# helenypzhang/Subspace-Multimodal-Learning

Hardware: AMD Instinct MI355X
Metric: bags/sec fwd+bwd, DeformCrossTransMIL N=10k x 512 (higher is better)
Workload: dtype f32

## Files before the change

subspace-multimodal-learning_amd/csrc/cpb_regions.h:

```cpp
#pragma once
#include <type_traits>
#include "deform_common.h"
#include "deform16_types.h"

namespace {

constexpr int RG_MAX_KEYS = 16384;
constexpr int RG_G = 1024;
constexpr int RG_SUB = 8;
constexpr int RG_SUBC = (RG_SUB + 1) * (RG_SUB + 1);
constexpr int RG_SUBCAP = 16384;
constexpr int RG_EDGES = 1 << 15;
constexpr unsigned RG_E_SUB0 = 4096u, RG_E_EDGE0 = RG_E_SUB0 + 16384u;
constexpr int RG_CANDCAP = 1 << 18;
constexpr int RG_HASH = 16384;
constexpr int RG_RCAP = 4096;
constexpr int RG_LCAP = 2048;
constexpr unsigned RG_NONE = 0xFFFFu;
constexpr unsigned long long RG_EMPTY = ~0ull;
constexpr unsigned RG_K_REGION = 0u << 30, RG_K_EDGE = 1u << 30, RG_K_SUB = 2u << 30, RG_K_MLP = 3u << 30, RG_PAYLOAD = 0x3FFFFFFFu;

struct RegionHeader {
  unsigned n_sub, n_edge, n_cand, n_regions, n_keys, overflow;
  unsigned n_cand1, pad0;
// ... 714 lines not shown
        for (int r = 0; r < 16; ++r) LTb[(size_t)(j0 + acc_row(r, hf)) * 32 + c] = s[r];
      } else {
#pragma unroll
        for (int r = 0; r < 16; ++r) {
          const int key = acc_row(r, hf);
          if (key < nk) LTb[(size_t)(j0 + key) * 32 + c] = s[r];
        }
      }
    }
    if constexpr (SAVE && !F32) {
      if (nk == KT) {
#pragma unroll
        for (int r = 0; r < 16; r += 2) {
          unsigned w = pack_score(s[r], s[r + 1]);
          if (dc.thresh) w = stash_keep16x2(w, keepbits >> r);
          const unsigned lo = w & 0xFFFFu, hi = w >> 16;
          LTb[(size_t)(j0 + acc_row(r, hf)) * 32 + c] = (u16)lo;
          LTb[(size_t)(j0 + acc_row(r + 1, hf)) * 32 + c] = (u16)hi;
          s[r] = score_of(lo); s[r + 1] = score_of(hi);
        }
      } else {
#pragma unroll
        for (int r = 0; r < 16; r += 2) {
          const unsigned w = pack_score(s[r], s[r + 1]);
          unsigned lo = w & 0xFFFFu, hi = w >> 16;
          const int k0 = acc_row(r, hf), k1 = acc_row(r + 1, hf);
          if (dc.thresh) {
            if (k0 < nk) lo = stash_keep16(lo, (keepbits >> r) & 1u);
            if (k1 < nk) hi = stash_keep16(hi, (keepbits >> (r + 1)) & 1u);
          }
          if (k0 < nk) { LTb[(size_t)(j0 + k0) * 32 + c] = (u16)lo; s[r] = score_of(lo); }
          if (k1 < nk) { LTb[(size_t)(j0 + k1) * 32 + c] = (u16)hi; s[r + 1] = score_of(hi); }
        }
      }
      tmax = -INFINITY;
#pragma unroll
      for (int r = 0; r < 16; ++r) tmax = fmaxf(tmax, s[r]);
    }
    fetch_kv(j0 + KT);
    if (kt + 1 < ntiles) step1((kt + 1) & 1);
    tmax = xhalf_max(tmax);
    const float m_new = fmaxf(m_run, tmax);
    const float alpha = sexp(m_run - m_new);
    float psum = 0.f;
#pragma unroll
    for (int r = 0; r < 16; ++r) {
      const float p = sexp(s[r] - m_new);
      psum += p;
      s[r] = p;
    }
    if (dc.thresh) {
#pragma unroll
      for (int r = 0; r < 16; ++r) s[r] *= ((keepbits >> r) & 1u) ? dc.keep_scale : 0.f;
    }
    l_run = l_run * alpha + psum;
    m_run = m_new;
#pragma unroll
    for (int r = 0; r < 16; ++r) { oacc0[r] *= alpha; oacc1[r] *= alpha; }
    if (kt + 1 < ntiles) step2a();
    __builtin_amdgcn_sched_barrier(0);

#pragma unroll
    for (int kb = 0; kb < 2; ++kb) {
      float p8[8];
#pragma unroll
      for (int j = 0; j < 8; ++j) p8[j] = s[8 * kb + j];
      const int ro = (16 * kb + 4 * hf + trq) * FTLD + trc;
      if constexpr (F32) {
        half8 ph, pl;
        split8(p8, ph, pl);
        const half8 vh0 = lds_frag_tr_h(&Vp[0][ro], &Vp[0][ro + 8 * FTLD]), vl0 = lds_frag_tr_h(&Vp[1][ro], &Vp[1][ro + 8 * FTLD]);
        const half8 vh1 = lds_frag_tr_h(&Vp[0][ro + 32], &Vp[0][ro + 32 + 8 * FTLD]), vl1 = lds_frag_tr_h(&Vp[1][ro + 32], &Vp[1][ro + 32 + 8 * FTLD]);
        oacc0 = mfma16(vl0, ph, oacc0); oacc0 = mfma16(vh0, pl, oacc0); oacc0 = mfma16(vh0, ph, oacc0);
        oacc1 = mfma16(vl1, ph, oacc1); oacc1 = mfma16(vh1, pl, oacc1); oacc1 = mfma16(vh1, ph, oacc1);
      } else {
        const vec8 pt = cvt8<T16>(p8);
        oacc0 = mma(frag_tr<T16>(&V16[ro], &V16[ro + 8 * FTLD]), pt, oacc0);
        oacc1 = mma(frag_tr<T16>(&V16[ro + 32], &V16[ro + 32 + 8 * FTLD]), pt, oacc1);
      }
    }
  }

  l_run = xhalf_sum(l_run);
  const float inv = 1.f / l_run;
  if (qvalid) {
    float* op = O + ((size_t)b * N + qi) * HD + h * DH;
#pragma unroll
    for (int rg = 0; rg < 4; ++rg) {
      const int d = 8 * rg + 4 * hf;
      *reinterpret_cast<float4*>(op + d) = make_float4(oacc0[4 * rg] * inv, oacc0[4 * rg + 1] * inv, oacc0[4 * rg + 2] * inv, oacc0[4 * rg + 3] * inv);
      *reinterpret_cast<float4*>(op + 32 + d) = make_float4(oacc1[4 * rg] * inv, oacc1[4 * rg + 1] * inv, oacc1[4 * rg + 2] * inv, oacc1[4 * rg + 3] * inv);
    }
    if (hf == 0) LSE[(size_t)(b * H + h) * N + qi] = m_run + logf(l_run);
  }
}

__device__ __forceinline__ long long region_fix(float v, double S) {
  return __double_as_longlong(fma((double)v, S, 6755399441055744.0)) - 0x4338000000000000ll;
}
struct RegionScale { double S; int e; };
__device__ __forceinline__ RegionScale region_scale(unsigned amax_bits, int kbits) {
  RegionScale r;
  r.e = amax_bits ? (int)((amax_bits >> 23) & 0xFFu) - 126 : 0;
  r.S = __longlong_as_double((long long)(1023 + kbits - r.e) << 52);
  return r;
}
constexpr int RG_GRAD = CPB_SLAB;

struct RegionBwdLds {
  unsigned long long hist[RG_LCAP * 3];
  unsigned long long grad[RG_GRAD];
  float2 reg2[RG_LCAP];
  float w2t[CH * CH], w2r[CH * CH];
  float2 dvs[16][64];
};

template <typename DS, bool MH = false>
__global__ __launch_bounds__(768) void cpb_region_bwd_kernel(
    const DS* __restrict__ dLT, const unsigned short* __restrict__ RID, const float* __restrict__ VS, const float* __restrict__ GQ,
    CpbParams cp, RegionView rv, const unsigned* __restrict__ AMAX, unsigned long long* __restrict__ HIST, unsigned long long* __restrict__ GRAD,
    float* __restrict__ dvs_slab, int N, int J, int H, int NST, int nkb, int nkbg, int chunks, int wpk, int tiles_per_chunk, int kbits, int shift,
    int lcap, int G) {
  extern __shared__ __attribute__((aligned(16))) unsigned char smem_raw[];
  RegionBwdLds& L = *reinterpret_cast<RegionBwdLds*>(smem_raw);
  const int tid = threadIdx.x, lane = tid & 63, c = lane & 31, hf = lane >> 5;
  const int wave = __builtin_amdgcn_readfirstlane(tid >> 6);
  const int b = blockIdx.z, h = blockIdx.y, chunk = blockIdx.x % chunks, grp = blockIdx.x / chunks;
  const int nthreads = blockDim.x;
  const int hpg = MH ? H / G : 1, g = MH ? h / hpg : h, oi = MH ? h - g * hpg : 0;
  const float4* __restrict__ regs = (MH && oi) ? region_reg1(rv.hdr) : rv.reg;
  HIST += MH ? (size_t)oi * RG_RCAP * 3 : 0;
  GRAD += MH ? (size_t)oi * RG_GRAD : 0;
  {
    const int nreg = min((int)rv.hdr->n_regions, lcap);
    for (int i = tid; i < RG_LCAP * 3; i += nthreads) L.hist[i] = 0ull;
    for (int i = tid; i < RG_GRAD; i += nthreads) L.grad[i] = 0ull;
    for (int i = tid; i < nreg; i += nthreads) { const float4 r = regs[i]; L.reg2[i] = make_float2(r.x, r.y); }
    for (int i = tid; i < CH * CH; i += nthreads) { const float w = cp.w2[i]; L.w2r[i] = w; L.w2t[(i & 31) * CH + (i >> 5)] = w; }
  }
  __syncthreads();
  const RegionScale sc = region_scale(*AMAX, kbits);
  const double Sg = __longlong_as_double(__double_as_longlong(sc.S) - ((long long)shift << 52));
  const CoopMlp mlp{cp.w1[c * 2], cp.w1[c * 2 + 1], cp.b1[c], cp.b2[c], cp.w3[oi * CH + c], cp.b3[oi], L.w2t, L.w2r};
  float big;
  asm("s_mov_b32 %0, 0x71800000" : "=s"(big));

  const int kb = grp * nkbg + __builtin_amdgcn_readfirstlane(wave % nkbg), tslot = __builtin_amdgcn_readfirstlane(wave / nkbg);
  const int key = lane * nkb + kb;
  const bool kvalid = key < J && kb < nkb;
  const int keyc = min(key, J - 1);
  const size_t vrow = (size_t)(b * (MH ? G : H) + g) * J;
  const float vs0 = VS[(vrow + keyc) * 2], vs1 = VS[(vrow + keyc) * 2 + 1];
  const int ntq = (N + QT - 1) / QT;
  const int t_begin = chunk * tiles_per_chunk, t_end = min(t_begin + tiles_per_chunk, ntq);
  float dv0 = 0.f, dv1 = 0.f;
  unsigned bad = 0u;
  unsigned cur = ~0u;
  float r0 = 0.f, r1 = 0.f, r2 = 0.f, u0 = 0.f, u1 = 0.f;
  typedef __attribute__((address_space(3))) unsigned long long lds_u64;
  typedef __attribute__((address_space(1))) unsigned long long glb_u64;
  lds_u64* const hist_l = (lds_u64*)L.hist;
  glb_u64* const hist_g = (glb_u64*)HIST;
  auto flush = [&]() {
    if (cur < (unsigned)lcap) {
      const float2 a = L.reg2[cur];
      dv0 = fmaf(-a.x, u0, dv0); dv1 = fmaf(-a.y, u1, dv1);
      lds_u64* hp = hist_l + cur * 3;
      __hip_atomic_fetch_add(hp, (unsigned long long)region_fix(r0, sc.S), __ATOMIC_RELAXED, __HIP_MEMORY_SCOPE_WORKGROUP);
      __hip_atomic_fetch_add(hp + 1, (unsigned long long)region_fix(r1, sc.S), __ATOMIC_RELAXED, __HIP_MEMORY_SCOPE_WORKGROUP);
      __hip_atomic_fetch_add(hp + 2, (unsigned long long)region_fix(r2, sc.S), __ATOMIC_RELAXED, __HIP_MEMORY_SCOPE_WORKGROUP);
    } else if (cur < (unsigned)RG_NONE) {
      const float4 a = regs[cur];
      dv0 = fmaf(-a.x, u0, dv0); dv1 = fmaf(-a.y, u1, dv1);
      glb_u64* hp = hist_g + cur * 3;
      __hip_atomic_fetch_add(hp, (unsigned long long)region_fix(r0, Sg), __ATOMIC_RELAXED, __HIP_MEMORY_SCOPE_AGENT);
      __hip_atomic_fetch_add(hp + 1, (unsigned long long)region_fix(r1, Sg), __ATOMIC_RELAXED, __HIP_MEMORY_SCOPE_AGENT);
      __hip_atomic_fetch_add(hp + 2, (unsigned long long)region_fix(r2, Sg), __ATOMIC_RELAXED, __HIP_MEMORY_SCOPE_AGENT);
    }
  };

  constexpr bool DS32 = std::is_same<DS, float>::value;
  float4 dbn[DS32 ? 8 : 4];
  uint4 ridn[4];
  float2 gqn;
  auto fetch = [&](int tile) {
    const size_t row = ((size_t)(b * H + h) * NST + (size_t)tile * QT) * J + (size_t)keyc * 32;
    const float4* dp = reinterpret_cast<const float4*>(dLT + row);
    const uint4* rp = reinterpret_cast<const uint4*>(RID + row);
#pragma unroll
    for (int i = 0; i < (DS32 ? 8 : 4); ++i) dbn[i] = dp[i];
#pragma unroll
    for (int i = 0; i < 4; ++i) ridn[i] = rp[i];
    gqn = reinterpret_cast<const float2*>(GQ)[min(tile * QT + c, N - 1)];
  };
  if (t_begin + tslot < t_end) fetch(t_begin + tslot);
  for (int tile = t_begin + tslot; tile < t_end; tile += wpk) {
    const int q0 = __builtin_amdgcn_readfirstlane(tile) * QT;
    const int nq = min(QT, N - q0);
    float dbr[32];
    unsigned ridw[16];
    if constexpr (DS32) {
#pragma unroll
      for (int i = 0; i < 8; ++i) { dbr[4 * i] = dbn[i].x; dbr[4 * i + 1] = dbn[i].y; dbr[4 * i + 2] = dbn[i].z; dbr[4 * i + 3] = dbn[i].w; }
    } else {
#pragma unroll
      for (int i = 0; i < 4; ++i) {
        const unsigned w4[4] = {__float_as_uint(dbn[i].x), __float_as_uint(dbn[i].y), __float_as_uint(dbn[i].z), __float_as_uint(dbn[i].w)};
#pragma unroll
        for (int j = 0; j < 4; ++j) { dbr[8 * i + 2 * j] = bf_lo(w4[j]); dbr[8 * i + 2 * j + 1] = bf_hi(w4[j]); }
      }
    }
#pragma unroll
    for (int i = 0; i < 4; ++i) { ridw[4 * i] = ridn[i].x; ridw[4 * i + 1] = ridn[i].y; ridw[4 * i + 2] = ridn[i].z; ridw[4 * i + 3] = ridn[i].w; }
    if (!kvalid) {
#pragma unroll
      for (int i = 0; i < 16; ++i) ridw[i] = 0xFFFFFFFFu;
    }
    const int gqx = __float_as_int(gqn.x), gqy = __float_as_int(gqn.y);
    if (tile + wpk < t_end) fetch(tile + wpk);
    unsigned nonemask = 0u;
    int gy_prev = 0;
    float p1 = 0.f, s1 = 0.f;
#pragma unroll
    for (int q = 0; q < 32; ++q) {
      if (q < nq) {
        const int gxb = __builtin_amdgcn_readlane(gqx, q), gyb = __builtin_amdgcn_readlane(gqy, q);
        const float d0 = __int_as_float(gxb) - vs0;
        const float p0 = slog1p(d0), s0 = dpos_of<false>(d0, big);
        if (q == 0 || gyb != gy_prev) {
          const float d1 = __int_as_float(gyb) - vs1;
          p1 = slog1p(d1); s1 = dpos_of<false>(d1, big);
          gy_prev = gyb;
        }
        const unsigned id = (ridw[q >> 1] >> (16 * (q & 1))) & 0xFFFFu;
        const float dbv = dbr[q];
        if constexpr (MH) {
          unsigned ub = __float_as_uint(dbv);
          asm("" : "+v"(ub));
          bad |= ((ub & 0x7F800000u) == 0x7F800000u) ? 1u : 0u;
        }
        if (id != cur) {
          flush();
          if (id == RG_NONE) { nonemask |= 1u << q; cur = ~0u; }
          else cur = id;
          r0 = 0.f; r1 = 0.f; r2 = 0.f; u0 = 0.f; u1 = 0.f;
        }
        r0 += dbv; r1 = fmaf(dbv, p0, r1); r2 = fmaf(dbv, p1, r2);
        u0 = fmaf(dbv, s0, u0); u1 = fmaf(dbv, s1, u1);
      }
    }
    if (!kvalid) nonemask = 0u;
    for (unsigned long long todo = __ballot(nonemask != 0u); todo; todo &= todo - 1) {
      const int l = __ffsll((long long)todo) - 1;
      const float v0 = __shfl(vs0, l), v1 = __shfl(vs1, l);
      const int kl = __shfl(keyc, l);
      const DS* drow = dLT + ((size_t)(b * H + h) * NST + (size_t)q0) * J + (size_t)kl * 32;
      for (unsigned m = (unsigned)__shfl((int)nonemask, l); m; m &= m - 1) {
        const int q = __ffs((int)m) - 1;
        const float d0 = GQ[(size_t)(q0 + q) * 2] - v0, d1 = GQ[(size_t)(q0 + q) * 2 + 1] - v1;
        const float pp0 = slog1p(d0), pp1 = slog1p(d1);
        float dbl;
        if constexpr (DS32) dbl = drow[q];
        else dbl = tof<__bf16>((unsigned)drow[q]);
        float h1; bool on2;
        (void)coop_mlp_fwd(mlp, pp0, pp1, c, h1, on2);
        float x2 = mlp.b2;
#pragma unroll 8
        for (int i = 0; i < CH; ++i) x2 = fmaf(mlp.w2t[i * CH + c], __shfl(h1, i), x2);
        const float g2 = on2 ? mlp.w3 : 0.f;
        float c1 = 0.f;
#pragma unroll 8
        for (int o = 0; o < CH; ++o) c1 = fmaf(mlp.w2r[o * CH + c], __shfl(g2, o), c1);
        c1 = h1 > 0.f ? c1 : 0.f;
        const float dp0 = coop_sum32(c1 * mlp.w1x), dp1 = coop_sum32(c1 * mlp.w1y);
        if (lane == l) {
          dv0 = fmaf(-dbl * dp0, dpos_of<false>(d0, big), dv0);
          dv1 = fmaf(-dbl * dp1, dpos_of<false>(d1, big), dv1);
        }
        for (int ii = 0; ii < 16; ++ii) {
          const int i = 16 * hf + ii;
          const float hi = __shfl(h1, i);
          atomicAdd(&L.grad[c * CH + i], (unsigned long long)region_fix(dbl * g2 * hi, sc.S));
        }
        if (hf == 0) {
          atomicAdd(&L.grad[1024 + 2 * c], (unsigned long long)region_fix(dbl * c1 * pp0, sc.S));
          atomicAdd(&L.grad[1024 + 2 * c + 1], (unsigned long long)region_fix(dbl * c1 * pp1, sc.S));
          atomicAdd(&L.grad[1024 + 64 + c], (unsigned long long)region_fix(dbl * c1, sc.S));
          atomicAdd(&L.grad[1024 + 96 + c], (unsigned long long)region_fix(dbl * g2, sc.S));
          atomicAdd(&L.grad[1024 + 128 + c], (unsigned long long)region_fix(on2 ? dbl * x2 : 0.f, sc.S));
          if (c == 0) atomicAdd(&L.grad[1024 + 160], (unsigned long long)region_fix(dbl, sc.S));
        }
      }
    }
  }
  flush();
  if constexpr (MH) {
    if (__ballot(kvalid && bad != 0u) && lane == 0) atomicOr(const_cast<unsigned*>(AMAX) + 1, 1u);
  }
  L.dvs[wave][lane] = make_float2(dv0, dv1);
  __syncthreads();
  if (wave < nkbg && kvalid) {
    float2 sum = L.dvs[wave][lane];
    for (int s2 = 1; s2 < wpk; ++s2) { const float2 t = L.dvs[wave + s2 * nkbg][lane]; sum.x += t.x; sum.y += t.y; }
    reinterpret_cast<float2*>(dvs_slab)[((size_t)chunk * gridDim.z * gridDim.y + (size_t)(b * H + h)) * J + key] = sum;
  }
  const long long half = shift > 0 ? (1ll << (shift - 1)) : 0ll;
  for (int i = tid; i < RG_LCAP * 3; i += nthreads) {
    const long long v = (long long)L.hist[i];
    if (v != 0ll) atomicAdd(&HIST[i], (unsigned long long)((v + half) >> shift));
  }
  for (int i = tid; i < RG_GRAD; i += nthreads) {
    const long long v = (long long)L.grad[i];
    if (v != 0ll) atomicAdd(&GRAD[i], (unsigned long long)((v + half) >> shift));
  }
}
template <typename T>
__global__ __launch_bounds__(256) void region_dvs_reduce_kernel(const T* __restrict__ slab, T* __restrict__ dVS, int H, int J, int chunks) {
  const int j = blockIdx.x * blockDim.x + threadIdx.x;
  if (j >= J) return;
  const int G = gridDim.y, hpg = H / G;
  const size_t per = (size_t)gridDim.z * H * J, first = ((size_t)blockIdx.z * H + blockIdx.y * hpg) * J + j;
  T s = slab[first];
  for (int k = 0; k < chunks; ++k)
    for (int o = k ? 0 : 1; o < hpg; ++o) s += slab[(size_t)k * per + first + (size_t)o * J];
  dVS[((size_t)blockIdx.z * G + blockIdx.y) * J + j] = s;
}

constexpr int RG_FIN = 32, RG_HPG = 2;
template <typename Geo, int HPG>
struct RegionSlab {
  static constexpr int W2 = 0, W1 = CH * CH, B1 = W1 + CH * Geo::PD, B2 = B1 + CH, W3 = B2 + CH, B3 = W3 + HPG * CH, N = B3 + HPG;
  static constexpr int STRIDE = N > RG_GRAD ? N : RG_GRAD;
};
struct Region2DGeo {
  typedef RegionTables Tables;
  typedef float2 Pos;
  static constexpr int PD = 2, W1 = WD_W1, B1 = WD_B1, W2 = WD_W2, B2 = WD_B2, GROUPS = RG_RCAP / RG_FIN;
  static constexpr bool DIRECT = true;
  __device__ static int w3(int o) { return o ? WD_W3B : WD_W3; }
  __device__ static int count(const Tables& t) { return (int)t.hdr->n_regions; }
  __device__ static double moment(const unsigned long long* HIST, int o, int r, int m) {
    return (double)(long long)HIST[((size_t)o * RG_RCAP + r) * 3 + m];
  }
  __device__ static double x1(const double* wd, int i, const double* M) {
    return wd[W1 + 2 * i] * M[1] + wd[W1 + 2 * i + 1] * M[2] + wd[B1 + i] * M[0];
  }
};
constexpr int RG_GRAD2 = RegionSlab<Region2DGeo, RG_HPG>::STRIDE;
static_assert(RegionSlab<Region2DGeo, 1>::N <= RG_GRAD && RG_GRAD2 > RG_GRAD, "gradient slabs");
__host__ __device__ inline int region_slab_stride(int hpg) { return hpg > 1 ? RG_GRAD2 : RG_GRAD; }

template <typename Geo, int HPG>
__global__ __launch_bounds__(256) void region_final1_kernel(typename Geo::Tables t, const unsigned long long* __restrict__ HIST,
                                                            double* __restrict__ part) {
  typedef RegionSlab<Geo, HPG> S;
  constexpr int NM = Geo::PD + 1;
  __shared__ double M[HPG][RG_FIN][NM], H1[HPG][RG_FIN][CH], X2[HPG][RG_FIN][CH], C1[HPG][RG_FIN][CH];
  __shared__ unsigned D1[RG_FIN], D2[RG_FIN];
  const int tid = threadIdx.x, r0 = blockIdx.x * RG_FIN;
  const int nreg = Geo::count(t);
  const double* __restrict__ wd = t.wd;
  for (int x = tid; x < HPG * RG_FIN * NM; x += 256) {
    const int o = x / (RG_FIN * NM), rr = (x / NM) % RG_FIN, m = x % NM, r = r0 + rr;
    M[o][rr][m] = r < nreg ? Geo::moment(HIST, o, r, m) : 0.0;
  }
  if (tid < RG_FIN) {
    const int r = r0 + tid;
    const unsigned long long k = r < nreg ? t.pat[r] : 0ull;
    D1[tid] = (unsigned)k; D2[tid] = (unsigned)(k >> 32);
  }
  __syncthreads();
  for (int x = tid; x < HPG * RG_FIN * CH; x += 256) {
    const int o = x / (RG_FIN * CH), r = (x >> 5) % RG_FIN, i = x & 31;
    H1[o][r][i] = ((D1[r] >> i) & 1u) ? Geo::x1(wd, i, M[o][r]) : 0.0;
  }
  __syncthreads();
  for (int x = tid; x < HPG * RG_FIN * CH; x += 256) {
    const int o = x / (RG_FIN * CH), r = (x >> 5) % RG_FIN, q = x & 31;
    double v = wd[Geo::B2 + q] * M[o][r][0];
    for (int i = 0; i < CH; ++i) v = fma(wd[Geo::W2 + q * CH + i], H1[o][r][i], v);
    X2[o][r][q] = v;
    double cc = 0.0;
    for (int qq = 0; qq < CH; ++qq)
      if ((D2[r] >> qq) & 1u) cc = fma(wd[Geo::W2 + qq * CH + q], wd[Geo::w3(o) + qq], cc);
    C1[o][r][q] = ((D1[r] >> q) & 1u) ? cc : 0.0;
  }
  __syncthreads();
  double* out = part + (size_t)blockIdx.x * S::STRIDE;
  for (int k = tid; k < S::N; k += 256) {
    double v = 0.0;
    for (int o = 0; o < HPG; ++o) {
      double s = 0.0;
      if (k < S::W1) {
        const int q = k >> 5, i = k & 31;
        for (int r = 0; r < RG_FIN; ++r) if ((D2[r] >> q) & 1u) s += H1[o][r][i];
        s *= wd[Geo::w3(o) + q];
      } else if (k < S::B1) {
        const int i = (k - S::W1) / Geo::PD, comp = (k - S::W1) % Geo::PD;
        for (int r = 0; r < RG_FIN; ++r) s = fma(C1[o][r][i], M[o][r][1 + comp], s);
      } else if (k < S::B2) {
        const int i = k - S::B1;
        for (int r = 0; r < RG_FIN; ++r) s = fma(C1[o][r][i], M[o][r][0], s);
      } else if (k < S::W3) {
        const int q = k - S::B2;
        for (int r = 0; r < RG_FIN; ++r) if ((D2[r] >> q) & 1u) s += M[o][r][0];
        s *= wd[Geo::w3(o) + q];
      } else if (k < S::B3) {
        const int q = (k - S::W3) & 31;
        if ((k - S::W3) >> 5 == o)
          for (int r = 0; r < RG_FIN; ++r) if ((D2[r] >> q) & 1u) s += X2[o][r][q];
      } else if (k - S::B3 == o) {
        for (int r = 0; r < RG_FIN; ++r) s += M[o][r][0];
      }
      v = o ? v + s : s;
    }
    out[k] = v;
  }
}
template <typename Geo, int HPG>
__global__ __launch_bounds__(256) void region_final2_kernel(const double* __restrict__ part, const unsigned long long* __restrict__ GRAD,
                                                            const unsigned* __restrict__ AMAX, int kbits_global, float* __restrict__ dW1,
                                                            float* __restrict__ db1, float* __restrict__ dW2, float* __restrict__ db2,
                                                            float* __restrict__ dW3, float* __restrict__ db3) {
  typedef RegionSlab<Geo, HPG> S;
  typedef RegionSlab<Geo, 1> S1;
  const int k = blockIdx.x * blockDim.x + threadIdx.x;
  if (k >= S::N) return;
  double v = 0.0;
  if constexpr (Geo::DIRECT) {
    unsigned long long gi;
    if (k < S::W3) {
      gi = GRAD[k];
      for (int o = 1; o < HPG; ++o) gi += GRAD[(size_t)o * RG_GRAD + k];
    } else if (k < S::B3) {
      gi = GRAD[(size_t)((k - S::W3) >> 5) * RG_GRAD + S1::W3 + ((k - S::W3) & 31)];
    } else {
      gi = GRAD[(size_t)(k - S::B3) * RG_GRAD + S1::B3];
    }
    v = (double)(long long)gi;
  }
  for (int g = 0; g < Geo::GROUPS; ++g) v += part[(size_t)g * S::STRIDE + k];
  const RegionScale sc = region_scale(*AMAX, kbits_global);
  const unsigned r = AMAX[1] ? 0x7FC00000u : __float_as_uint((float)(v / sc.S));
  auto put = [&](float* dst, int i) { reinterpret_cast<unsigned*>(dst)[i] = r; };
  if (k < S::W1) put(dW2, k);
  else if (k < S::B1) put(dW1, k - S::W1);
  else if (k < S::B2) put(db1, k - S::B1);
  else if (k < S::W3) put(db2, k - S::B2);
  else if (k < S::B3) put(dW3, k - S::W3);
  else put(db3, k - S::B3);
}

static int ceil_log2_u64(unsigned long long x) { int k = 0; while ((1ull << k) < x && k < 63) ++k; return k; }
struct RegionBwdPlan {
  int chunks, tiles_per_chunk, nkb, nkbg, ngrp, wpk, kbits, shift;
  size_t amax, hist, grad, dvs, part, total;
};
static RegionBwdPlan region_bwd_plan(int B, int N, int J, int H, int outputs = 1) {
  RegionBwdPlan p;
  const int ntq = (N + QT - 1) / QT;
  p.chunks = (512 + B * H - 1) / (B * H);
  if (p.chunks < 1) p.chunks = 1;
  if (p.chunks > ntq) p.chunks = ntq;
  p.tiles_per_chunk = (ntq + p.chunks - 1) / p.chunks;
  p.chunks = (ntq + p.tiles_per_chunk - 1) / p.tiles_per_chunk;
  p.nkb = (J + 63) / 64;
  p.ngrp = (p.nkb + 11) / 12;
  p.nkbg = (p.nkb + p.ngrp - 1) / p.ngrp;
  p.wpk = 12 / p.nkbg;
  if (p.wpk > p.tiles_per_chunk) p.wpk = p.tiles_per_chunk;
  const int kl = 60 - ceil_log2_u64((unsigned long long)p.tiles_per_chunk * QT * J) - 2;
  const int kg = 60 - ceil_log2_u64((unsigned long long)B * H * N * J) - 2;
  p.kbits = kl < 38 ? kl : 38;
  const int kgl = kg < p.kbits ? kg : p.kbits;
  p.shift = p.kbits - kgl;
  size_t o = (bwd_workspace(B, N, J, H).total * sizeof(float) + 255) & ~(size_t)255;
  auto take = [&](size_t bytes) { const size_t at = o; o += (bytes + 255) & ~(size_t)255; return at; };
  p.amax = take(256);
  p.hist = take((size_t)outputs * RG_RCAP * 3 * 8);
  p.grad = take((size_t)outputs * RG_GRAD * 8);
  p.dvs = take((size_t)p.chunks * B * H * J * 2 * sizeof(float));
  p.part = take((size_t)(RG_RCAP / RG_FIN) * region_slab_stride(outputs) * 8);
  p.total = o;
  return p;
}

static int check_region(const char* fn, int B, int N, int J, int H, int G, bool dims_first = false) {
  SMML_REQUIRE(G > 0 && !(dims_first && (B <= 0 || N <= 0 || J <= 0 || H <= 0)), "%s: non-positive dimension", fn);
  SMML_REQUIRE(H > 0 && H % G == 0 && H / G <= RG_HPG, "%s: heads (%d) must be 1 or 2 per offset group (%d groups)", fn, H, G);
  SMML_REQUIRE(B > 0 && N > 0 && J > 0, "%s: non-positive dimension", fn);
  SMML_REQUIRE(deform_dims_ok(B, N, J, H), "%s: B, H <= 65535, N <= 2^26, J <= 2^22 (got B %d N %d J %d H %d)", fn, B, N, J, H);
  SMML_REQUIRE(J <= RG_MAX_KEYS, "%s: the region kernels take at most %d keys (got %d)", fn, RG_MAX_KEYS, J);
  return SMML_OK;
}
static int check_region_workspace(const char* fn, const void* ws, size_t bytes, const RegionBwdPlan& pl, int J) {
  if (int rc = check_workspace(fn, ws, bytes, pl.total, 256)) return rc;
  SMML_REQUIRE(pl.wpk >= 1, "%s: too many keys (%d)", fn, J);
  return SMML_OK;
}
static int region_lcap(const SmmlDeformOpts* opts) {
  return (opts && opts->region_lds_cap > 0) ? (opts->region_lds_cap < RG_LCAP ? opts->region_lds_cap : RG_LCAP) : RG_LCAP;
}


template <typename Geo>
static void region_final_launch(typename Geo::Tables t, char* wsb, const RegionBwdPlan& pl, int B, int J, int H, int G, float* dvs, float* dw1,
                                float* db1, float* dw2, float* db2, float* dw3, float* db3, hipStream_t st) {
  typedef typename Geo::Pos Pos;
  const unsigned* amax = reinterpret_cast<const unsigned*>(wsb + pl.amax);
  const unsigned long long* hist = reinterpret_cast<const unsigned long long*>(wsb + pl.hist);
  const unsigned long long* grad = reinterpret_cast<const unsigned long long*>(wsb + pl.grad);
  double* part = reinterpret_cast<double*>(wsb + pl.part);
  hipLaunchKernelGGL(region_dvs_reduce_kernel<Pos>, dim3((J + 255) / 256, G, B), dim3(256), 0, st, reinterpret_cast<const Pos*>(wsb + pl.dvs),
                     reinterpret_cast<Pos*>(dvs), H, J, pl.chunks);
  auto finals = [&](auto hpg) {
    constexpr int HPG = decltype(hpg)::value;
    hipLaunchKernelGGL((region_final1_kernel<Geo, HPG>), dim3(Geo::GROUPS), dim3(256), 0, st, t, hist, part);
    hipLaunchKernelGGL((region_final2_kernel<Geo, HPG>), dim3((RegionSlab<Geo, HPG>::N + 255) / 256), dim3(256), 0, st, part, grad, amax,
                       pl.kbits - pl.shift, dw1, db1, dw2, db2, dw3, db3);
  };
  if (H / G == 2) finals(std::integral_constant<int, 2>());
  else finals(std::integral_constant<int, 1>());
}

template <typename DS, bool MH = false>
static int region_bias_bwd_launch(const char* fn, const DS* dlogits, const unsigned short* region_ids, const float* vs, const float* gq, CpbParams cp,
                                  const void* tables, char* wsb, const RegionBwdPlan& pl, int B, int N, int J, int H, int G, int nst, int lcap,
                                  float* dvs, float* dw1, float* db1, float* dw2, float* db2, float* dw3, float* db3, void* ev_start, void* ev_stop,
                                  hipStream_t st) {
  const RegionView rv = region_view(const_cast<void*>(tables));
  unsigned* amax = reinterpret_cast<unsigned*>(wsb + pl.amax);
  unsigned long long* hist = reinterpret_cast<unsigned long long*>(wsb + pl.hist);
  unsigned long long* grad = reinterpret_cast<unsigned long long*>(wsb + pl.grad);
  float* dvs_slab = reinterpret_cast<float*>(wsb + pl.dvs);
  {
    const hipError_t e = hipFuncSetAttribute(reinterpret_cast<const void*>(cpb_region_bwd_kernel<DS, MH>),
                                             hipFuncAttributeMaxDynamicSharedMemorySize, (int)sizeof(RegionBwdLds));
    SMML_REQUIRE(e == hipSuccess, "%s: hipFuncSetAttribute failed: %s", fn, hipGetErrorString(e));
  }
  if (ev_start) (void)hipEventRecord((hipEvent_t)ev_start, st);
  hipLaunchKernelGGL((cpb_region_bwd_kernel<DS, MH>), dim3(pl.chunks * pl.ngrp, H, B), dim3(64 * pl.nkbg * pl.wpk), sizeof(RegionBwdLds), st, dlogits,
                     region_ids, vs, gq, cp, rv, amax, hist, grad, dvs_slab, N, J, H, nst, pl.nkb, pl.nkbg, pl.chunks, pl.wpk, pl.tiles_per_chunk,
                     pl.kbits, pl.shift, lcap, G);
  if (ev_stop) (void)hipEventRecord((hipEvent_t)ev_stop, st);
  SMML_LAUNCH_CHECK(fn);
  region_final_launch<Region2DGeo>(region_tables(const_cast<void*>(tables)), wsb, pl, B, J, H, G, dvs, dw1, db1, dw2, db2, dw3, db3, st);
  SMML_LAUNCH_CHECK(fn);
  return SMML_OK;
}

}
```

subspace-multimodal-learning_amd/csrc/deform_attn.hip:

```cpp
#include "deform_common.h"
#include "cpb_regions.h"
#include "cpb_regions1d.h"

namespace {


constexpr int FWD_WPS = 2;
template <int PDX, bool SAVE>
__global__ __launch_bounds__(256, FWD_WPS) void deform_attn_fwd_kernel(
    const float* __restrict__ Q, const float* __restrict__ K, const float* __restrict__ V,
    const float* __restrict__ VS, const float* __restrict__ GQ, CpbParams cp, float* __restrict__ O,
    float* __restrict__ LSE, float* __restrict__ LT, unsigned short* __restrict__ MK, int N, int J, int H, int G, int NST,
    float scale, DropCfg dc_in) {
  constexpr int PD = PosCfg<PDX>::PD;
  constexpr bool RAW = PosCfg<PDX>::RAW;
  const DropCfg dc = drop_resolve(dc_in);
  __shared__ __attribute__((aligned(16))) _Float16 Kp[2][KT * FRLD];
  __shared__ __attribute__((aligned(16))) _Float16 Vp[2][KT * FTLD];
  __shared__ __attribute__((aligned(16))) _Float16 Qp[WAVES][2][QT * FRLD];
  __shared__ float vsl[KT][2];
  __shared__ float biasT[WAVES][KT][QT];

  const int tid = threadIdx.x, wave = tid >> 6, lane = tid & 63, c = lane & 31, hf = lane >> 5;
  const int b = blockIdx.z, h = blockIdx.y;
// ... 228 lines not shown
  const bool qvalid = (q0 + c) < N;
  const int qi = qvalid ? (q0 + c) : (N - 1);

  bf16x8 doh[4], dom[4], dol[4];
  float delta = 0.f;
  {
    const size_t off = ((size_t)b * N + qi) * HD + h * DH + hf * 8;
#pragma unroll
    for (int kb = 0; kb < 4; ++kb) {
      const float4 t0 = *reinterpret_cast<const float4*>(dO + off + 16 * kb), t1 = *reinterpret_cast<const float4*>(dO + off + 16 * kb + 4);
      const float4 u0 = *reinterpret_cast<const float4*>(O + off + 16 * kb), u1 = *reinterpret_cast<const float4*>(O + off + 16 * kb + 4);
      delta += t0.x * u0.x + t0.y * u0.y + t0.z * u0.z + t0.w * u0.w + t1.x * u1.x + t1.y * u1.y + t1.z * u1.z + t1.w * u1.w;
      const float x8[8] = {t0.x, t0.y, t0.z, t0.w, t1.x, t1.y, t1.z, t1.w};
      split8_bf3(x8, doh[kb], dom[kb], dol[kb]);
    }
  }
  delta = xhalf_sum(delta);
  const float nl = prob_bias(LSE[(size_t)(b * H + h) * N + qi]);

  floatx16 dq0 = {0}, dq1 = {0};
  float amax = 0.f;
  float rho = 0.f;
  const float* Kb = K + (size_t)b * J * HD + h * DH;
  const float* Vb = V + (size_t)b * J * HD + h * DH;
  const float* LTb = LT + ((size_t)(b * H + h) * NST + q0) * J;
  float* dLTb = dLT + ((size_t)(b * H + h) * NST + q0) * J;

  const int skey = tid >> 4, sd4 = (tid & 15) * 4;
  const int trq = (lane & 15) >> 2, trc = 16 * ((lane >> 4) & 1) + 4 * (lane & 3);
  float4 kreg[2], vreg[2];
  float lt[16];
  auto fetch = [&](int j0, float4 (&kr)[2], float4 (&vr)[2], float (&l)[16]) {
#pragma unroll
    for (int i = 0; i < 2; ++i) {
      const int key = j0 + skey + 16 * i;
      kr[i] = make_float4(0.f, 0.f, 0.f, 0.f); vr[i] = kr[i];
      if (key < J) {
        kr[i] = *reinterpret_cast<const float4*>(Kb + (size_t)key * HD + sd4);
        vr[i] = *reinterpret_cast<const float4*>(Vb + (size_t)key * HD + sd4);
      }
    }
#pragma unroll
    for (int r = 0; r < 16; ++r) {
      const int key = min(j0 + acc_row(r, hf), J - 1);
      l[r] = LTb[(size_t)key * 32 + c];
    }
  };
  fetch(0, kreg, vreg, lt);

  const int ntiles = (J + KT - 1) / KT;
  for (int kt = 0; kt < ntiles; ++kt) {
    const int j0 = kt * KT, buf = kt & 1;
    const int nk = min(KT, J - j0);
#pragma unroll
    for (int i = 0; i < 2; ++i) {
      const int key = skey + 16 * i;
      uint2v hh, mm, ll;
      split4_bf3(vreg[i], hh, mm, ll);
      *reinterpret_cast<uint2v*>(&Vp[buf][0][key * VBLD + sd4]) = hh;
      *reinterpret_cast<uint2v*>(&Vp[buf][1][key * VBLD + sd4]) = mm;
      *reinterpret_cast<uint2v*>(&Vp[buf][2][key * VBLD + sd4]) = ll;
      split4_bf3(kreg[i], hh, mm, ll);
      *reinterpret_cast<uint2v*>(&Kp[buf][0][key * KBLD + sd4]) = hh;
      *reinterpret_cast<uint2v*>(&Kp[buf][1][key * KBLD + sd4]) = mm;
    }
    __syncthreads();
    float ltc[16];
#pragma unroll
    for (int r = 0; r < 16; ++r) ltc[r] = lt[r];
    if (kt + 1 < ntiles) fetch(j0 + KT, kreg, vreg, lt);

    floatx16 dp = {0};
#pragma unroll
    for (int kb = 0; kb < 4; ++kb) {
      const int o = c * VBLD + 16 * kb + 8 * hf;
      const bf16x8 vh = *reinterpret_cast<const bf16x8*>(&Vp[buf][0][o]);
      const bf16x8 vm = *reinterpret_cast<const bf16x8*>(&Vp[buf][1][o]);
      const bf16x8 vl = *reinterpret_cast<const bf16x8*>(&Vp[buf][2][o]);
      dp = bwd_prod<3>(vh, vm, vl, doh[kb], dom[kb], dol[kb], dp);
    }

    float ds[16];
    if (nk == KT && q0 + QT <= N) {
#pragma unroll
      for (int r = 0; r < 16; ++r) {
        const float p = prob_of(ltc[r], nl);
        float dpr = dp[r];
        if (dc.thresh) dpr *= stashed_factor(ltc[r], dc.keep_scale);
        const float v = p * (dpr - delta);
        dLTb[(size_t)(j0 + acc_row(r, hf)) * 32 + c] = v;
        ds[r] = v;
        rho += v;
        amax = fmaxf(amax, fabsf(v));
      }
    } else {
#pragma unroll
      for (int r = 0; r < 16; ++r) {
        const int key = acc_row(r, hf);
        float v = 0.f;
        if (key < nk && qvalid) {
          const float p = prob_of(ltc[r], nl);
          float dpr = dp[r];
          if (dc.thresh) dpr *= stashed_factor(ltc[r], dc.keep_scale);
          v = p * (dpr - delta);
          dLTb[(size_t)(j0 + key) * 32 + c] = v;
        }
        ds[r] = v;
        rho += v;
        amax = fmaxf(amax, fabsf(v));
      }
    }
#pragma unroll
    for (int kb = 0; kb < 2; ++kb) {
      float x8[8];
#pragma unroll
      for (int jx = 0; jx < 8; ++jx) x8[jx] = ds[8 * kb + jx];
      bf16x8 sh, sm, sl;
      split8_bf3(x8, sh, sm, sl);
      const int ro = (16 * kb + 4 * hf + trq) * KBLD + trc;
#pragma unroll
      for (int db = 0; db < 2; ++db) {
        const bf16x8 kh = lds_frag_tr(&Kp[buf][0][ro + 32 * db], &Kp[buf][0][ro + 32 * db + 8 * KBLD]);
        const bf16x8 km = lds_frag_tr(&Kp[buf][1][ro + 32 * db], &Kp[buf][1][ro + 32 * db + 8 * KBLD]);
        if (db == 0) dq0 = bwd_prod<2>(kh, km, km, sh, sm, sm, dq0);
        else dq1 = bwd_prod<2>(kh, km, km, sh, sm, sm, dq1);
      }
    }
  }
  rho = xhalf_sum(rho);
  if (qvalid && hf == 0) RHO[(size_t)(b * H + h) * N + qi] = rho;
  if (AMAX) {
    amax = wave_max_all(amax);
    if (lane == 0 && amax > 0.f) atomicMax(AMAX, __float_as_uint(amax));
  }
  if (qvalid) {
    float* qp = dQ + ((size_t)b * N + qi) * HD + h * DH;
#pragma unroll
    for (int rg = 0; rg < 4; ++rg) {
      const int d = 8 * rg + 4 * hf;
      *reinterpret_cast<float4*>(qp + d) = make_float4(dq0[4 * rg] * scale, dq0[4 * rg + 1] * scale,
                                                       dq0[4 * rg + 2] * scale, dq0[4 * rg + 3] * scale);
      *reinterpret_cast<float4*>(qp + 32 + d) = make_float4(dq1[4 * rg] * scale, dq1[4 * rg + 1] * scale,
                                                            dq1[4 * rg + 2] * scale, dq1[4 * rg + 3] * scale);
    }
  }
}


__global__ __launch_bounds__(256, 2) void deform_attn_bwd_dkv_kernel(
    const float* __restrict__ Q, const float* __restrict__ dO, const float* __restrict__ LSE,
    const float* __restrict__ LT, const float* __restrict__ dLT, float* __restrict__ dKp,
    float* __restrict__ dVp, int N, int J, int H, int NST, int nkg, int tiles_per_part, int nparts, int Bn, DropCfg dc_in) {
  const DropCfg dc = drop_resolve(dc_in);
  __shared__ __attribute__((aligned(16))) __bf16 Qp[2][3][QT * QBLD];
  __shared__ __attribute__((aligned(16))) __bf16 dOp[2][3][QT * QBLD];
  __shared__ __attribute__((aligned(16))) float nls[2][QT];
  const int tid = threadIdx.x, wave = tid >> 6, lane = tid & 63, c = lane & 31, hf = lane >> 5;
  const int nslices = nparts * H * Bn;
  const int chunk = blockIdx.x / (8 * nkg), rem = blockIdx.x - chunk * (8 * nkg);
  const int kg = rem >> 3, slice = chunk * 8 + (rem & 7);
  if (slice >= nslices) return;
  const int part = slice % nparts, h = (slice / nparts) % H, b = slice / (nparts * H);
  const int j0 = kg * DKV_KEYS + wave * KT;
  const int HD = H * DH;
  const int nk = min(KT, J - j0);
  const bool kvalid = c < nk;
  const int key = min(j0 + c, J - 1);
  const float* LTk = LT + (size_t)(b * H + h) * NST * J + (size_t)key * 32;
  const float* dLTk = dLT + (size_t)(b * H + h) * NST * J + (size_t)key * 32;
  const float* LSEb = LSE + (size_t)(b * H + h) * N;

  const int nqt = (N + QT - 1) / QT;
  const int qt_begin = part * tiles_per_part, qt_end = min(qt_begin + tiles_per_part, nqt);

  const int srow = tid >> 4, sd4 = (tid & 15) * 4;
  const int trq = (lane & 15) >> 2, trc = 16 * ((lane >> 4) & 1) + 4 * (lane & 3);
  float4 qreg[2], doreg[2], ltr[4], dlr[4];
  float lsereg = 0.f;
#pragma unroll
  for (int i = 0; i < 4; ++i) { ltr[i] = make_float4(0.f, 0.f, 0.f, 0.f); dlr[i] = ltr[i]; qreg[i >> 1] = ltr[i]; doreg[i >> 1] = ltr[i]; }
  auto fetch = [&](int q0) {
#pragma unroll
    for (int i = 0; i < 2; ++i) {
      const int qrow = min(q0 + srow + 16 * i, N - 1);
      const size_t off = ((size_t)b * N + qrow) * HD + h * DH + sd4;
      qreg[i] = *reinterpret_cast<const float4*>(Q + off);
      doreg[i] = *reinterpret_cast<const float4*>(dO + off);
    }
#pragma unroll
    for (int rg = 0; rg < 4; ++rg) {
      const size_t qq = (size_t)q0 * J + 8 * rg + 4 * hf;
      ltr[rg] = *reinterpret_cast<const float4*>(LTk + qq);
      dlr[rg] = *reinterpret_cast<const float4*>(dLTk + qq);
    }
    if (tid < QT) lsereg = LSEb[min(q0 + tid, N - 1)];
  };

  floatx16 dk0 = {0}, dk1 = {0}, dv0 = {0}, dv1 = {0};
  if (qt_begin < qt_end) fetch(qt_begin * QT);
  for (int qt = qt_begin; qt < qt_end; ++qt) {
    const int q0 = qt * QT, buf = (qt - qt_begin) & 1;
#pragma unroll
    for (int i = 0; i < 2; ++i) {
      const int o = (srow + 16 * i) * QBLD + sd4;
      uint2v hh, mm, ll;
      split4_bf3(qreg[i], hh, mm, ll);
      *reinterpret_cast<uint2v*>(&Qp[buf][0][o]) = hh;
      *reinterpret_cast<uint2v*>(&Qp[buf][1][o]) = mm;
      split4_bf3(doreg[i], hh, mm, ll);
      *reinterpret_cast<uint2v*>(&dOp[buf][0][o]) = hh;
      *reinterpret_cast<uint2v*>(&dOp[buf][1][o]) = mm;
    }
    if (tid < QT) nls[buf][tid] = prob_bias(lsereg);
    __syncthreads();
    float lv[16], dsv[16], ls[16];
#pragma unroll
    for (int rg = 0; rg < 4; ++rg) {
      lv[4 * rg + 0] = ltr[rg].x; lv[4 * rg + 1] = ltr[rg].y; lv[4 * rg + 2] = ltr[rg].z; lv[4 * rg + 3] = ltr[rg].w;
      dsv[4 * rg + 0] = dlr[rg].x; dsv[4 * rg + 1] = dlr[rg].y; dsv[4 * rg + 2] = dlr[rg].z; dsv[4 * rg + 3] = dlr[rg].w;
      const float4 t = *reinterpret_cast<const float4*>(&nls[buf][8 * rg + 4 * hf]);
      ls[4 * rg + 0] = t.x; ls[4 * rg + 1] = t.y; ls[4 * rg + 2] = t.z; ls[4 * rg + 3] = t.w;
    }
    if (qt + 1 < qt_end) fetch(q0 + QT);
    if (nk > 0) {
      float p[16], ds[16];
      if (nk == KT && q0 + QT <= N) {
#pragma unroll
        for (int r = 0; r < 16; ++r) {
          float pv = prob_of(lv[r], ls[r]);
          if (dc.thresh) pv *= stashed_factor(lv[r], dc.keep_scale);
          p[r] = pv; ds[r] = dsv[r];
        }
      } else {
#pragma unroll
        for (int r = 0; r < 16; ++r) {
          const int qq = q0 + acc_row(r, hf);
          const bool ok = kvalid && qq < N;
          float pv = ok ? prob_of(lv[r], ls[r]) : 0.f;
          if (dc.thresh && ok) pv *= stashed_factor(lv[r], dc.keep_scale);
          p[r] = pv;
          ds[r] = ok ? dsv[r] : 0.f;
        }
      }
#pragma unroll
      for (int kb = 0; kb < 2; ++kb) {
        float x8[8], y8[8];
#pragma unroll
        for (int jx = 0; jx < 8; ++jx) { x8[jx] = p[8 * kb + jx]; y8[jx] = ds[8 * kb + jx]; }
        bf16x8 ph, pm, pl, sh, sm, sl;
        split8_bf3(x8, ph, pm, pl);
        split8_bf3(y8, sh, sm, sl);
        const int ro = (16 * kb + 4 * hf + trq) * QBLD + trc;
#pragma unroll
        for (int db = 0; db < 2; ++db) {
          const int o = ro + 32 * db;
          const bf16x8 ah = lds_frag_tr(&dOp[buf][0][o], &dOp[buf][0][o + 8 * QBLD]);
          const bf16x8 am = lds_frag_tr(&dOp[buf][1][o], &dOp[buf][1][o + 8 * QBLD]);
          const bf16x8 qh = lds_frag_tr(&Qp[buf][0][o], &Qp[buf][0][o + 8 * QBLD]);
          const bf16x8 qm = lds_frag_tr(&Qp[buf][1][o], &Qp[buf][1][o + 8 * QBLD]);
          if (db == 0) { dv0 = bwd_prod<2>(ah, am, am, ph, pm, pm, dv0); dk0 = bwd_prod<2>(qh, qm, qm, sh, sm, sm, dk0); }
          else { dv1 = bwd_prod<2>(ah, am, am, ph, pm, pm, dv1); dk1 = bwd_prod<2>(qh, qm, qm, sh, sm, sm, dk1); }
        }
      }
    }
  }
  if (kvalid) {
    const size_t off = (((size_t)part * Bn + b) * J + (j0 + c)) * HD + h * DH;
    float* kp = dKp + off;
    float* vp = dVp + off;
#pragma unroll
    for (int rg = 0; rg < 4; ++rg) {
      const int d = 8 * rg + 4 * hf;
      *reinterpret_cast<float4*>(kp + d) = make_float4(dk0[4 * rg], dk0[4 * rg + 1], dk0[4 * rg + 2], dk0[4 * rg + 3]);
      *reinterpret_cast<float4*>(kp + 32 + d) = make_float4(dk1[4 * rg], dk1[4 * rg + 1], dk1[4 * rg + 2], dk1[4 * rg + 3]);
      *reinterpret_cast<float4*>(vp + d) = make_float4(dv0[4 * rg], dv0[4 * rg + 1], dv0[4 * rg + 2], dv0[4 * rg + 3]);
      *reinterpret_cast<float4*>(vp + 32 + d) = make_float4(dv1[4 * rg], dv1[4 * rg + 1], dv1[4 * rg + 2], dv1[4 * rg + 3]);
    }
  }
}


template <int PDX>
__global__ __launch_bounds__(256, 2) void cpb_bwd_kernel(
    const float* __restrict__ dLT, const unsigned short* __restrict__ MK, const float* __restrict__ LT,
    const float* __restrict__ LSE, const float* __restrict__ RHO, const float* __restrict__ VS,
    const float* __restrict__ GQ, CpbParams cp, float* __restrict__ slab, float* __restrict__ dvs_slab, int N, int J, int H,
    int G, int NST) {
  constexpr int PD = PosCfg<PDX>::PD;
  constexpr bool RAW = PosCfg<PDX>::RAW;
  extern __shared__ __attribute__((aligned(16))) float smem[];
  const int tid = threadIdx.x, wave = tid >> 6, lane = tid & 63, c = lane & 31, hf = lane >> 5;
  const int b = blockIdx.z, h = blockIdx.y;
  const int q0 = blockIdx.x * (QT * WAVES) + wave * QT;
  const int o = H / G, g = h / o, oi = h - g * o;
  const bool qvalid = (q0 + c) < N;
  const int qi = qvalid ? (q0 + c) : (N - 1);

  float* tab = smem;
  float* wbase = smem + CPB2_TAB;
  float* xq = wbase + wave * CPB2_WAVE_LDS;
  float2* stg = reinterpret_cast<float2*>(xq + CPB_XQ);
  const int wg = (blockIdx.z * gridDim.y + blockIdx.y) * gridDim.x + blockIdx.x;
  float2* dvs_row = reinterpret_cast<float2*>(dvs_slab) + (size_t)(wg * WAVES + wave) * J;
  if (tid < 32) {
    const int ch = acc_row(tid & 15, tid >> 4);
    tab[(tid >> 4) * 32 + (tid & 15)] = cp.w1[ch * PD];
    tab[(tid >> 4) * 32 + 16 + (tid & 15)] = (PD == 2) ? cp.w1[ch * PD + 1] : 0.f;
  }
// ... 608 lines not shown
```

Measured before the change: 1235.

## Size region backward grid to CU count and skip idle key-block waves

Region backward planning now queries the device CU count. It splits key blocks into groups using divisors of the key-block count, then picks the number of query-tile chunks that best fills whole rounds of workgroups across the CUs, up to a cap. Waves whose key block is past the end now get an empty tile range, so they do no loop work. Separately, the dKV kernel's bf16 Q and dO staging buffers drop from three slots to two, cutting LDS use, which could raise occupancy. The risks are more chunks, which means more partial-sum traffic, and out-of-bounds indexing if any code still uses the third staging slot.

```diff
diff --git a/subspace-multimodal-learning_amd/csrc/cpb_regions.h b/subspace-multimodal-learning_amd/csrc/cpb_regions.h
--- a/subspace-multimodal-learning_amd/csrc/cpb_regions.h
+++ b/subspace-multimodal-learning_amd/csrc/cpb_regions.h
@@ -890,7 +890,7 @@
   const size_t vrow = (size_t)(b * (MH ? G : H) + g) * J;
   const float vs0 = VS[(vrow + keyc) * 2], vs1 = VS[(vrow + keyc) * 2 + 1];
   const int ntq = (N + QT - 1) / QT;
-  const int t_begin = chunk * tiles_per_chunk, t_end = min(t_begin + tiles_per_chunk, ntq);
+  const int t_begin = chunk * tiles_per_chunk, t_end = kb < nkb ? min(t_begin + tiles_per_chunk, ntq) : t_begin;
   float dv0 = 0.f, dv1 = 0.f;
   unsigned bad = 0u;
   unsigned cur = ~0u;
@@ -1190,6 +1190,19 @@
 }
 
 static int ceil_log2_u64(unsigned long long x) { int k = 0; while ((1ull << k) < x && k < 63) ++k; return k; }
+constexpr double REGION_BWD_FILL = 0.9;
+constexpr int REGION_BWD_MAX_CHUNKS = 64;
+static int region_bwd_cus() {
+  static const int cus = [] {
+    int dev = 0, n = 0;
+    if (hipGetDevice(&dev) != hipSuccess || hipDeviceGetAttribute(&n, hipDeviceAttributeMultiprocessorCount, dev) != hipSuccess || n <= 0) {
+      (void)hipGetLastError();
+      n = 256;
+    }
+    return n;
+  }();
+  return cus;
+}
 struct RegionBwdPlan {
   int chunks, tiles_per_chunk, nkb, nkbg, ngrp, wpk, kbits, shift;
   size_t amax, hist, grad, dvs, part, total;
@@ -1197,15 +1210,25 @@
 static RegionBwdPlan region_bwd_plan(int B, int N, int J, int H, int outputs = 1) {
   RegionBwdPlan p;
   const int ntq = (N + QT - 1) / QT;
-  p.chunks = (512 + B * H - 1) / (B * H);
-  if (p.chunks < 1) p.chunks = 1;
-  if (p.chunks > ntq) p.chunks = ntq;
+  p.nkb = (J + 63) / 64;
+  p.nkbg = 1;
+  for (const int c : {12, 6, 4, 3, 2})
+    if (p.nkb % c == 0) { p.nkbg = c; break; }
+  p.ngrp = p.nkb / p.nkbg;
+  p.wpk = 12 / p.nkbg;
+  const long long base = (long long)p.ngrp * B * H, cus = region_bwd_cus();
+  const int cmax = ntq / p.wpk < 1 ? 1 : (ntq / p.wpk < REGION_BWD_MAX_CHUNKS ? ntq / p.wpk : REGION_BWD_MAX_CHUNKS);
+  double best_occ = -1.0;
+  p.chunks = 1;
+  for (int c = 1; c <= cmax; ++c) {
+    const int tpc = (ntq + c - 1) / c, eff = (ntq + tpc - 1) / tpc;
+    const long long wg = eff * base, rounds = (wg + cus - 1) / cus;
+    const double occ = (double)wg / (double)(rounds * cus);
+    if (occ > best_occ + 1e-9) { best_occ = occ; p.chunks = eff; }
+    if (occ >= REGION_BWD_FILL) { p.chunks = eff; break; }
+  }
   p.tiles_per_chunk = (ntq + p.chunks - 1) / p.chunks;
   p.chunks = (ntq + p.tiles_per_chunk - 1) / p.tiles_per_chunk;
-  p.nkb = (J + 63) / 64;
-  p.ngrp = (p.nkb + 11) / 12;
-  p.nkbg = (p.nkb + p.ngrp - 1) / p.ngrp;
-  p.wpk = 12 / p.nkbg;
   if (p.wpk > p.tiles_per_chunk) p.wpk = p.tiles_per_chunk;
   const int kl = 60 - ceil_log2_u64((unsigned long long)p.tiles_per_chunk * QT * J) - 2;
   const int kg = 60 - ceil_log2_u64((unsigned long long)B * H * N * J) - 2;
diff --git a/subspace-multimodal-learning_amd/csrc/deform_attn.hip b/subspace-multimodal-learning_amd/csrc/deform_attn.hip
--- a/subspace-multimodal-learning_amd/csrc/deform_attn.hip
+++ b/subspace-multimodal-learning_amd/csrc/deform_attn.hip
@@ -404,8 +404,8 @@
     const float* __restrict__ LT, const float* __restrict__ dLT, float* __restrict__ dKp,
     float* __restrict__ dVp, int N, int J, int H, int NST, int nkg, int tiles_per_part, int nparts, int Bn, DropCfg dc_in) {
   const DropCfg dc = drop_resolve(dc_in);
-  __shared__ __attribute__((aligned(16))) __bf16 Qp[2][3][QT * QBLD];
-  __shared__ __attribute__((aligned(16))) __bf16 dOp[2][3][QT * QBLD];
+  __shared__ __attribute__((aligned(16))) __bf16 Qp[2][2][QT * QBLD];
+  __shared__ __attribute__((aligned(16))) __bf16 dOp[2][2][QT * QBLD];
   __shared__ __attribute__((aligned(16))) float nls[2][QT];
   const int tid = threadIdx.x, wave = tid >> 6, lane = tid & 63, c = lane & 31, hf = lane >> 5;
   const int nslices = nparts * H * Bn;
```

New measurement: 1248, median of 6. 1.01x the previous value.
